# nghorbani/moshpp

Hardware: NVIDIA H100
Metric: mocap frames solved/sec (Stage-II) (higher is better)
Workload: dtype f32

## Files before the change

### moshpp_b200/csrc/mosh2_device.cuh

```cuda
#pragma once
#include <math.h>
#include <stdint.h>

#if defined(__CUDACC__) && !defined(MOSH2_EMU)
#define M2_HD __host__ __device__ __forceinline__
#define M2_D __device__ __forceinline__
#define M2_NOINLINE __device__ __noinline__
#define M2_SYNC() __syncthreads()
#define M2_WSYNC() __syncwarp()
#define M2_GPU 1
#else
#define M2_HD inline
#define M2_D inline
#define M2_NOINLINE static inline
#define M2_SYNC() ((void)0)
#define M2_WSYNC() ((void)0)
#define M2_GPU 0
#endif

#if defined(MOSH2_PROFILE) && M2_GPU
#define M2_T0() long long t_prev_ = clock64()
#define M2_TACC(slot) do { if (cta.tid == 0) { const long long t_now_ = clock64(); w.prof[(slot) + prof_base] += t_now_ - t_prev_; t_prev_ = t_now_; } } while (0)
#define M2_TRESET() do { t_prev_ = clock64(); } while (0)
#else
// ... 1450 lines not shown
                real sacc = on ? s0 + s1 : real(0);
                const real a1 = __shfl_sync(0xffffffffu, sacc, (src0 + 1) & 31), a2 = __shfl_sync(0xffffffffu, sacc, (src0 + 2) & 31);
                if (on && part == 0) out[i] = (sacc + a1) + a2;
            }
        }
        __syncthreads();
#else
        for (int i = 0; i < n; ++i) {
            real s = 0;
            for (int j = 0; j < n; ++j) s += w.A[i * d.lda + j] * v[j];
            out[i] = s;
        }
#endif
    }

    M2_D bool chol_diag(int k0, int n) {
        const int ld = d.ld;
        constexpr int NB = kCholNB;
        const int kb = (n - k0 < NB) ? n - k0 : NB;
        real *Li = w.Linv + (k0 / NB) * NB * NB;
#if M2_GPU
        {

            const int lane = cta.tid;
            real *base = w.Lm + (k0 * ld + k0);
            real Lb[NB][NB], invd[NB], x[NB];
#pragma unroll
            for (int r = 0; r < NB; ++r) {
                Vec4<real> v0, v1;
                v0.x = v0.y = v0.z = v0.w = real(0);
                v1 = v0;
                if (r < kb) {
                    v0 = ld4(base + r * ld);
                    if (r >= 4) v1 = ld4(base + r * ld + 4);
                } else {
                    if (r == 0) v0.x = real(1);
                    if (r == 1) v0.y = real(1);
                    if (r == 2) v0.z = real(1);
                    if (r == 3) v0.w = real(1);
                    if (r == 4) v1.x = real(1);
                    if (r == 5) v1.y = real(1);
                    if (r == 6) v1.z = real(1);
                    if (r == 7) v1.w = real(1);
                }
                Lb[r][0] = v0.x; Lb[r][1] = v0.y; Lb[r][2] = v0.z; Lb[r][3] = v0.w;
                Lb[r][4] = v1.x; Lb[r][5] = v1.y; Lb[r][6] = v1.z; Lb[r][7] = v1.w;
            }
            bool ok = true;
#pragma unroll
            for (int cc = 0; cc < NB; ++cc) {
                const real piv = Lb[cc][cc];
                if (!(piv > pivot_eps<real>())) ok = false;
                const real iv = r_rsqrt(piv);
                Lb[cc][cc] = piv * iv;
                invd[cc] = iv;
#pragma unroll
                for (int r = cc + 1; r < NB; ++r) Lb[r][cc] *= iv;
#pragma unroll
                for (int r = cc + 1; r < NB; ++r)
#pragma unroll
                    for (int q = cc + 1; q <= r; ++q) Lb[r][q] -= Lb[r][cc] * Lb[q][cc];
            }
            const int c = lane & (NB - 1);
#pragma unroll
            for (int r = 0; r < NB; ++r) x[r] = (r == c) ? real(1) : real(0);
#pragma unroll
            for (int pp = 0; pp < NB; ++pp) {
                x[pp] *= invd[pp];
#pragma unroll
                for (int r = pp + 1; r < NB; ++r) x[r] -= Lb[r][pp] * x[pp];
            }
            if (lane < NB) {
#pragma unroll
                for (int r = 0; r < NB; ++r) Li[r * NB + lane] = x[r];
            }
            __syncwarp();
            if (lane == 0) {
#pragma unroll
                for (int r = 0; r < NB; ++r)
                    if (r < kb) {
                        Vec4<real> v0, v1;
                        v0.x = Lb[r][0]; v0.y = r >= 1 ? Lb[r][1] : real(0); v0.z = r >= 2 ? Lb[r][2] : real(0); v0.w = r >= 3 ? Lb[r][3] : real(0);
                        *reinterpret_cast<Vec4<real> *>(base + r * ld) = v0;
                        if (r >= 4) {
                            v1.x = Lb[r][4]; v1.y = r >= 5 ? Lb[r][5] : real(0); v1.z = r >= 6 ? Lb[r][6] : real(0); v1.w = r >= 7 ? Lb[r][7] : real(0);
                            *reinterpret_cast<Vec4<real> *>(base + r * ld + 4) = v1;
                        }
                    }
            }
            return ok;
                }
#else
        {

            real Lk[NB * NB], id[NB];
            bool ok = true;
            for (int r = 0; r < kb; ++r)
                for (int cc = 0; cc <= r; ++cc) {
                    real sacc = w.Lm[(k0 + r) * ld + k0 + cc];
                    for (int p = 0; p < cc; ++p) sacc -= Lk[r * NB + p] * Lk[cc * NB + p];
                    if (cc == r) {
                        if (!(sacc > pivot_eps<real>())) { ok = false; sacc = real(1); }
                        const real sq = r_sqrt(sacc);
                        Lk[r * NB + r] = sq;
                        id[r] = real(1) / sq;
                    } else Lk[r * NB + cc] = sacc * id[cc];
                }
            for (int cc = 0; cc < kb; ++cc)
                for (int r = 0; r < kb; ++r) {
                    real v = 0;
                    if (r == cc) v = id[r];
                    else if (r > cc) {
                        real sacc = 0;
                        for (int p = cc; p < r; ++p) sacc -= Lk[r * NB + p] * Li[p * NB + cc];
                        v = sacc * id[r];
                    }
                    Li[r * NB + cc] = v;
                }
            for (int r = 0; r < kb; ++r)
                for (int cc = 0; cc <= r; ++cc) w.Lm[(k0 + r) * ld + k0 + cc] = Lk[r * NB + cc];
            for (int r = 0; r < NB; ++r)
                for (int cc = 0; cc < NB; ++cc)
                    if (r >= kb || cc >= kb) Li[r * NB + cc] = (r == cc) ? real(1) : real(0);
            if (!ok) w.isc[3] = 0;
            return ok;
                }
#endif
    }

    M2_D void chol_tile(int it, int r0, int n) {
        const int ld = d.ld;
        constexpr int NB = kCholNB;
        int ti = 0, rem = it;
        while (rem > ti) { rem -= ti + 1; ++ti; }
        const int tj = rem;
        real acc[kBS * kBS];
#pragma unroll
        for (int q = 0; q < kBS * kBS; ++q) acc[q] = 0;
#pragma unroll
        for (int cc = 0; cc < NB; ++cc) {
            const Vec4<real> av = ld4(w.Pn + cc * d.ldp + r0 + ti * kBS), bv = ld4(w.Pn + cc * d.ldp + r0 + tj * kBS);
            const real ai[4] = {av.x, av.y, av.z, av.w}, bj[4] = {bv.x, bv.y, bv.z, bv.w};
#pragma unroll
            for (int p = 0; p < kBS; ++p)
#pragma unroll
                for (int q = 0; q < kBS; ++q) acc[p * kBS + q] += ai[p] * bj[q];
        }
#pragma unroll
        for (int p = 0; p < kBS; ++p) {
            const int i = r0 + ti * kBS + p;
            if (i <= n && r0 + tj * kBS < n) {
                real *dst = w.Lm + i * ld + r0 + tj * kBS;
                Vec4<real> v = ld4(dst);
                v.x -= acc[p * kBS]; v.y -= acc[p * kBS + 1]; v.z -= acc[p * kBS + 2]; v.w -= acc[p * kBS + 3];
                *reinterpret_cast<Vec4<real> *>(dst) = v;
            }
        }
    }

    M2_D void panel_row(int i, int k0, int kb, const real *Li, int n) {
        const int ld = d.ld;
        constexpr int NB = kCholNB;
        real xr[NB];
#pragma unroll
        for (int cc = 0; cc < NB; ++cc) xr[cc] = 0;
        if (i <= n) {
            real *row = w.Lm + i * ld + k0;
            real av[NB];
            {
                const Vec4<real> a0 = ld4(row), a1 = ld4(row + 4);
                av[0] = a0.x; av[1] = a0.y; av[2] = a0.z; av[3] = a0.w; av[4] = a1.x; av[5] = a1.y; av[6] = a1.z; av[7] = a1.w;
            }
#pragma unroll
            for (int cc = 0; cc < NB; ++cc) if (cc >= kb) av[cc] = real(0);
#pragma unroll
            for (int cc = 0; cc < NB; ++cc) {
                const Vec4<real> l0 = ld4(Li + cc * NB);
                real sacc = av[0] * l0.x;
                if (cc >= 1) sacc += av[1] * l0.y;
                if (cc >= 2) sacc += av[2] * l0.z;
                if (cc >= 3) sacc += av[3] * l0.w;
                if (cc >= 4) {
                    const Vec4<real> l1 = ld4(Li + cc * NB + 4);
                    sacc += av[4] * l1.x;
                    if (cc >= 5) sacc += av[5] * l1.y;
                    if (cc >= 6) sacc += av[6] * l1.z;
                    if (cc >= 7) sacc += av[7] * l1.w;
                }
                xr[cc] = cc < kb ? sacc : real(0);
            }
            if (kb == NB) {
                Vec4<real> o0, o1;
                o0.x = xr[0]; o0.y = xr[1]; o0.z = xr[2]; o0.w = xr[3]; o1.x = xr[4]; o1.y = xr[5]; o1.z = xr[6]; o1.w = xr[7];
                *reinterpret_cast<Vec4<real> *>(row) = o0;
                *reinterpret_cast<Vec4<real> *>(row + 4) = o1;
            } else {
#pragma unroll
                for (int cc = 0; cc < NB; ++cc) if (cc < kb) row[cc] = xr[cc];
            }
        }
#pragma unroll
        for (int cc = 0; cc < NB; ++cc) w.Pn[cc * d.ldp + i] = xr[cc];
    }

    M2_D bool gauss_newton(int n) {
        const int ld = d.ld;
        constexpr int NB = kCholNB;
        M2_T0();
        CTA_FOR(i, n) {
            const real a = w.A[i * d.lda + i];
            w.ds[i] = (a > real(0)) ? real(1) / r_sqrt(a) : real(0);
        }
        M2_SYNC();
#if M2_GPU
        {
            const int lane = cta.tid & 31, warp = cta.tid >> 5, nwarp = cta.nthr >> 5;
            for (int i = warp; i < n; i += nwarp)
                for (int j = lane; j <= i; j += 32) w.Lm[i * ld + j] = w.A[i * d.lda + j] * w.ds[i] * w.ds[j];
        }
#else
        for (int i = 0; i < n; ++i)
            for (int j = 0; j <= i; ++j) w.Lm[i * ld + j] = w.A[i * d.lda + j] * w.ds[i] * w.ds[j];
#endif
        CTA_FOR(j, n) w.Lm[n * ld + j] = w.g[j] * w.ds[j];
        M2_SYNC();
        M2_TACC(11);
#if M2_GPU
        {
            const int nthr = cta.nthr;
#pragma unroll 1
            for (int k0 = -NB; k0 < n; k0 += NB) {
                bool ok = true;
                const int kb = k0 < 0 ? 0 : ((n - k0 < NB) ? n - k0 : NB);
                const int r0 = k0 < 0 ? 0 : k0 + kb;
                const real *Li = w.Linv + (k0 < 0 ? 0 : k0 / NB) * NB * NB;
                const bool trail = k0 >= 0 && r0 < n;
                if (cta.tid < 32) {
                    if (k0 >= 0) {
                        const int i = r0 + cta.tid;
                        M2_TACC(14);
                        if (cta.tid < NB && i < d.ldp) panel_row(i, k0, kb, Li, n);
                        if (trail) {
                            __threadfence_block();
                            __syncwarp();
                            asm volatile("bar.arrive 1, %0;" :: "r"(nthr) : "memory");
                            {
                                const int pr = cta.tid >> 2, q0 = (cta.tid & 3) * 2;
                                const int ii = r0 + pr, jj = r0 + q0;
                                if (ii <= n && jj < n) {
                                    real acc0 = 0, acc1 = 0;
#pragma unroll
                                    for (int cc = 0; cc < NB; ++cc) {
                                        const real pi = w.Pn[cc * d.ldp + ii];
                                        acc0 += pi * w.Pn[cc * d.ldp + jj];
                                        acc1 += pi * w.Pn[cc * d.ldp + jj + 1];
                                    }
                                    w.Lm[ii * ld + jj] -= acc0;
                                    w.Lm[ii * ld + jj + 1] -= acc1;
                                }
                            }
                            __syncwarp();
                        }
                    }
                    M2_TACC(12);
                    if (r0 < n) ok = chol_diag(r0, n);
                    M2_TACC(13);
                } else {
                    if (k0 >= 0) {
                        const int t = cta.tid - 32, nt_ = nthr - 32;
                        for (int i = r0 + NB + t; i < d.ldp; i += nt_) panel_row(i, k0, kb, Li, n);
                        if (trail) {
                            asm volatile("bar.sync 1, %0;" :: "r"(nthr) : "memory");
                            const int R = n + 1 - r0, ntl = (R + kBS - 1) / kBS, ntri = ntl * (ntl + 1) / 2;
                            for (int it = 3 + t; it < ntri; it += nt_) chol_tile(it, r0, n);
                        }
                    }
                }
                if (__syncthreads_or(!ok)) return false;
            }
            M2_TACC(14);
        }
#else
        w.isc[3] = 1;
        chol_diag(0, n);
        if (w.isc[3] == 0) return false;
        for (int k0 = 0; k0 < n; k0 += NB) {
            const int kb = (n - k0 < NB) ? n - k0 : NB;
            const real *Li = w.Linv + (k0 / NB) * NB * NB;
            for (int i = k0 + kb; i < d.ldp; ++i) panel_row(i, k0, kb, Li, n);
            const int r0 = k0 + kb, R = r0 < n ? n + 1 - r0 : 0;
            if (R > 0) {
                const int nt = (R + kBS - 1) / kBS, ntri = nt * (nt + 1) / 2;
                for (int it = 0; it < ntri; ++it) chol_tile(it, r0, n);
                chol_diag(r0, n);
                if (w.isc[3] == 0) return false;
            }
        }
#endif
#if M2_GPU
        if (cta.tid < 128) {
            const int tid = cta.tid;
            for (int i = tid; i < n; i += 128) w.tmp[i] = w.Lm[n * ld + i];
            asm volatile("bar.sync 2, 128;" ::: "memory");
#pragma unroll 1
            for (int k0 = ((n - 1) / NB) * NB; k0 >= 0; k0 -= NB) {
                const int kb = (n - k0 < NB) ? n - k0 : NB;
                const real *Li = w.Linv + (k0 / NB) * NB * NB;
                real zv[NB], y[NB], Lr[NB][NB];
                {
                    const Vec4<real> z0 = ld4(w.tmp + k0), z1 = ld4(w.tmp + k0 + 4);
                    zv[0] = z0.x; zv[1] = z0.y; zv[2] = z0.z; zv[3] = z0.w; zv[4] = z1.x; zv[5] = z1.y; zv[6] = z1.z; zv[7] = z1.w;
                }
#pragma unroll
                for (int cc = 1; cc < NB; ++cc) if (cc >= kb) zv[cc] = real(0);
#pragma unroll
                for (int pp = 0; pp < NB; ++pp) {
                    const Vec4<real> l0 = ld4(Li + pp * NB);
                    Lr[pp][0] = l0.x; Lr[pp][1] = l0.y; Lr[pp][2] = l0.z; Lr[pp][3] = l0.w;
                    if (pp >= 4) {
                        const Vec4<real> l1 = ld4(Li + pp * NB + 4);
                        Lr[pp][4] = l1.x; Lr[pp][5] = l1.y; Lr[pp][6] = l1.z; Lr[pp][7] = l1.w;
                    }
                }
#pragma unroll
                for (int cc = 0; cc < NB; ++cc) {
                    real sacc = 0;
#pragma unroll
                    for (int pp = cc; pp < NB; ++pp) sacc += Lr[pp][cc] * zv[pp];
                    y[cc] = sacc;
                }
                for (int i = tid; i < k0; i += 128) {
                    real zi = w.tmp[i];
#pragma unroll
                    for (int cc = 0; cc < NB; ++cc) if (cc < kb) zi -= w.Lm[(k0 + cc) * ld + i] * y[cc];
                    w.tmp[i] = zi;
                }
                asm volatile("bar.sync 2, 128;" ::: "memory");
                if (tid == 0) {
                    if (kb == NB) {
                        Vec4<real> o0, o1;
                        o0.x = y[0]; o0.y = y[1]; o0.z = y[2]; o0.w = y[3]; o1.x = y[4]; o1.y = y[5]; o1.z = y[6]; o1.w = y[7];
                        *reinterpret_cast<Vec4<real> *>(w.tmp + k0) = o0;
                        *reinterpret_cast<Vec4<real> *>(w.tmp + k0 + 4) = o1;
                    } else {
#pragma unroll
                        for (int cc = 0; cc < NB; ++cc) if (cc < kb) w.tmp[k0 + cc] = y[cc];
                    }
                }
            }
            asm volatile("bar.sync 2, 128;" ::: "memory");
            for (int i = tid; i < n; i += 128) w.dgn[i] = w.tmp[i] * w.ds[i];
        }
#else
        const int wl = cta.nthr < 32 ? cta.nthr : 32;
        if (cta.tid < wl) {
            const int lane = cta.tid;
            for (int i = lane; i < n; i += wl) w.tmp[i] = w.Lm[n * ld + i];
            M2_WSYNC();
            for (int k0 = ((n - 1) / NB) * NB; k0 >= 0; k0 -= NB) {
                const int kb = (n - k0 < NB) ? n - k0 : NB;
                const real *Li = w.Linv + (k0 / NB) * NB * NB;
                real zv[NB], y[NB];
#pragma unroll
                for (int cc = 0; cc < NB; ++cc) zv[cc] = cc < kb ? w.tmp[k0 + cc] : real(0);
#pragma unroll
                for (int cc = 0; cc < NB; ++cc) {
                    real sacc = 0;
#pragma unroll
                    for (int pp = cc; pp < NB; ++pp) sacc += Li[pp * NB + cc] * zv[pp];
                    y[cc] = sacc;
                }
                for (int i = lane; i < k0; i += wl) {
                    real zi = w.tmp[i];
#pragma unroll
                    for (int cc = 0; cc < NB; ++cc) if (cc < kb) zi -= w.Lm[(k0 + cc) * ld + i] * y[cc];
                    w.tmp[i] = zi;
                }
                M2_WSYNC();
                if (lane == 0) {
#pragma unroll
                    for (int cc = 0; cc < NB; ++cc) if (cc < kb) w.tmp[k0 + cc] = y[cc];
                }
                M2_WSYNC();
            }
            for (int i = lane; i < n; i += wl) w.dgn[i] = w.tmp[i] * w.ds[i];
        }
#endif
        M2_SYNC();
        M2_TACC(15);
        return true;
    }

    M2_D void stage_tables(int which) {
        const int *free = which ? static_cast<const int *>(w.c_free2) : static_cast<const int *>(w.c_free1);
        const int n = which ? m.n2 : m.n1;
        CTA_FOR(i, d.NX) w.colmap[i] = -1;
        CTA_FOR(i, d.nJ) w.jlist[i] = 0;
        M2_SYNC();
        CTA_FOR(i, n) {
            const int fv = free[i];
            w.colmap[fv] = i;
            int src;
            if (fv < 3) src = -1 - fv;
            else if (fv < 3 + m.body_dof) { src = fv - 3; w.jlist[(fv - 3) / 3] = 1; }
            else if (fv < 3 + d.PR) src = -4;
            else src = d.PF + (fv - 3 - d.PR);
            w.colsrc[i] = src;
        }
        M2_SYNC();
        if (cta.tid == 0) {
            int hf = 0;
            for (int b = 0; b < m.hb_n; ++b) {
                bool any = false;
                for (int r = m.hb[b].r0; r < m.hb[b].r1; ++r) any = any || w.colmap[3 + m.body_dof + r] >= 0;
                if (any) {
                    hf = 1;
                    for (int q = m.hb[b].q0; q < m.hb[b].q1; ++q) w.jlist[(m.body_dof + q) / 3] = 1;
                }
            }
            int cnt = 0;
            for (int j = 0; j < d.nJ; ++j) if (w.jlist[j]) w.jlist[cnt++] = j;
            w.st_meta[2 * which] = cnt;
            w.st_meta[2 * which + 1] = hf;
        }
        M2_SYNC();
        CTA_FOR(i, d.NX) w.st_colmap[which * d.NX + i] = w.colmap[i];
        CTA_FOR(i, n) w.st_colsrc[which * d.n2 + i] = w.colsrc[i];
        CTA_FOR(i, d.nJ) w.st_jlist[which * d.nJ + i] = w.jlist[i];
        M2_SYNC();
    }

    M2_D void stage_setup(const StepCfg<real> &c) {
        ++n_min;
        const int which = c.free == static_cast<const int *>(w.c_free2) ? 1 : 0;
        CTA_FOR(i, d.NX) w.colmap[i] = w.st_colmap[which * d.NX + i];
        CTA_FOR(i, c.n) w.colsrc[i] = w.st_colsrc[which * d.n2 + i];
        CTA_FOR(i, d.nJ) w.jlist[i] = w.st_jlist[which * d.nJ + i];
        njl = w.st_meta[2 * which];
        hand_free = w.st_meta[2 * which + 1] != 0;
        M2_SYNC();
    }

    M2_D void solve_frame(int f, bool emit, bool first, bool fingers, bool dyn, bool face, bool light) {
        const Options &o = job.opt;
        const real e1 = real(1e-15), e2 = real(1e-15);
        enum { OP_PROCRUSTES, OP_BEGIN, OP_TRIAL, OP_OUTPUT };
        int op = first ? OP_PROCRUSTES : OP_BEGIN;
        int stage = first ? 0 : (light ? 4 : 3);
        if (lin_f >= 0) stage = job.lin_step == 2 ? 4 : 3;
        const int maxit = light ? 1 : o.maxiter;
        StepCfg<real> c;
        c.free = w.c_free1; c.n = m.n1; c.velo = has_velo; c.poseH = false; c.dm_terms = false; c.extrap = false; c.face = false;
        c.wp = 0; c.e3 = real(o.e3_first);
        bool need_setup = !first;
        real sse0 = 0, delta = 0, alpha = 0, nsd = 0, ngn2 = 0, gn_sd = 0, nstep = 0, npn = 0, gd = 0, dAd = 0;
        bool done = false, in_iter = false, have_gn = false, gn_ok = true;
        int iter = 0;
        M2_T0();
        while (true) {
            if (need_setup) {
                M2_TACC(25);
                c.free = w.c_free1; c.n = m.n1; c.poseH = false; c.dm_terms = false; c.extrap = false; c.face = false;
                if (stage < 3) {
                    c.wp = wp_frame * (stage == 0 ? real(10) : (stage == 1 ? real(5) : real(1)));
                    c.e3 = real(o.e3_first);
                } else {
                    c.wp = wp_frame;
                    c.e3 = real(o.e3);
                    if (stage == 4) { c.free = w.c_free2; c.n = m.n2; c.poseH = fingers; c.dm_terms = dyn; c.extrap = has_extrap; c.face = face; }
                }
                stage_setup(c);
                need_setup = false;
                M2_TACC(20);
            }
            const int n = c.n;
            {
                const bool reuse = op != OP_TRIAL && fwd_at_x && (fwd_has_prior || !(c.wp > real(0)));
                M2_TACC(25);
                eval(op == OP_TRIAL ? w.xt : w.x, c, reuse);
                M2_TRESET();
                if (!reuse) fwd_has_prior = c.wp > real(0);
                fwd_at_x = op != OP_TRIAL;
            }
            if (lin_f >= 0) {
                CTA_FOR(i, 3 * d.M) { job.markers_sim[size_t(f) * 3 * d.M + i] = w.mk[i]; if (job.lin_r) job.lin_r[size_t(f) * 3 * d.M + i] = w.rm[i]; }
                CTA_FOR(i, N_ERR) job.errs[size_t(f) * N_ERR + i] = w.sc[1 + i];
                if (job.lin_vp) CTA_FOR(i, 3 * d.S) job.lin_vp[size_t(f) * 3 * d.S + i] = w.vp[i];
                if (job.lin_mode < 2) break;
            }
            if (op == OP_PROCRUSTES) {
                procrustes();
                fwd_at_x = false;
                op = OP_BEGIN;
                need_setup = true;
                continue;
            }
            if (op == OP_OUTPUT) break;
            bool do_build = false, improved = false;
            if (op == OP_BEGIN) {
                sse0 = w.sc[0];
                delta = real(o.delta_0);
                done = false; in_iter = false; iter = 0;
                do_build = true;
            } else {
                const real sse1 = w.sc[0];
                real rho = sse0 - sse1;
                improved = rho > real(0) || rho >= -accept_slack<real>() * sse0;
                if (rho > real(0)) rho = rho / (real(2) * gd - dAd);
                if (improved) {
                    CTA_FOR(i, d.NX) w.x[i] = w.xt[i];
                    fwd_at_x = true;
                    M2_SYNC();
                    if (c.e3 > real(0) && (sse0 - sse1) / sse0 < c.e3) done = true;
                    else { do_build = true; sse0 = sse1; }
                }
                if (rho > real(0.9)) { const real cand = real(2.5) * nstep; if (cand > delta) delta = cand; }
                else if (rho < real(0.05)) delta *= real(0.25);
                if (delta <= e2 * npn) done = true;
                if (done || improved) {
                    in_iter = false;
                    if (!done && iter >= maxit) { done = true; if (!light) frame_flags |= ST_MAXITER; }
                }
            }
            M2_TACC(21);
            if (do_build && !done) build(w.x, c);
            M2_TRESET();
            if (lin_f >= 0) {
                CTA_FOR(idx, n * n) { const int i = idx / n, j = idx - i * n; job.lin_A[size_t(f) * n * n + idx] = w.A[i * d.lda + j]; }
                CTA_FOR(i, n) job.lin_g[size_t(f) * n + i] = w.g[i];
                break;
            }
            if (op == OP_BEGIN) {
                real sq[1] = {0};
                CTA_FOR(i, n) sq[0] += w.g[i] * w.g[i];
                cta_reduce<real, 1>(cta, sq, w.red);
                if (r_sqrt(sq[0]) < e1) done = true;
            }
            if (!done) {
                if (!in_iter) {
                    ++iter;
                    ++n_iter;
                    symv(w.g, w.Ag, n);
                    real r2[2] = {0, 0};
                    CTA_FOR(i, n) { r2[0] += w.g[i] * w.g[i]; r2[1] += w.g[i] * w.Ag[i]; }
                    cta_reduce<real, 2>(cta, r2, w.red);
                    alpha = r2[0] / r2[1];
                    nsd = alpha * r_sqrt(r2[0]);
                    have_gn = false; gn_ok = true;
                    in_iter = true;
                }
                int kind;
                real beta = 0, scale_sd = 0;
                if (nsd >= delta) { kind = 0; scale_sd = delta / nsd * alpha; }
                else {
                    if (!have_gn) {
                        M2_TACC(22);
                        gn_ok = gauss_newton(n);
                        M2_TRESET();
                        have_gn = true;
                        if (gn_ok) {
                            real q[2] = {0, 0};
                            CTA_FOR(i, n) { q[0] += w.dgn[i] * w.dgn[i]; q[1] += w.dgn[i] * w.g[i]; }
                            cta_reduce<real, 2>(cta, q, w.red);
                            ngn2 = q[0];
                            gn_sd = alpha * q[1];
                        } else frame_flags |= ST_GN_FALLBACK;
                    }
                    if (!gn_ok) { kind = 0; scale_sd = alpha; }
                    else if (r_sqrt(ngn2) <= delta) kind = 1;
                    else {
                        kind = 2;
                        const real dsq = delta * delta, sd2 = nsd * nsd;
                        const real diff2 = ngn2 - real(2) * gn_sd + sd2;
                        const real pnow = diff2 * dsq + gn_sd * gn_sd - ngn2 * sd2;
                        beta = (dsq - sd2) / ((gn_sd - sd2) + r_sqrt(pnow));
                    }
                }
                CTA_FOR(i, n) {
                    real v;
                    if (kind == 0) v = scale_sd * w.g[i];
                    else if (kind == 1) v = w.dgn[i];
                    else v = alpha * w.g[i] + beta * (w.dgn[i] - alpha * w.g[i]);
                    w.d[i] = v;
                }
                M2_SYNC();
                symv(w.d, w.tmp, n);
                real q[4] = {0, 0, 0, 0};
                CTA_FOR(i, n) {
                    q[0] += w.d[i] * w.d[i];
                    q[1] += w.g[i] * w.d[i];
                    q[2] += w.d[i] * w.tmp[i];
                    const real pv = w.x[c.free[i]];
                    q[3] += pv * pv;
                }
                cta_reduce<real, 4>(cta, q, w.red);
                nstep = r_sqrt(q[0]); gd = q[1]; dAd = q[2]; npn = r_sqrt(q[3]);
                if (nstep <= e2 * npn) done = true;
                else {
                    CTA_FOR(i, d.NX) w.xt[i] = w.x[i];
                    M2_SYNC();
                    CTA_FOR(i, n) w.xt[c.free[i]] += w.d[i];
                    M2_SYNC();
                    op = OP_TRIAL;
                    M2_TACC(23);
                    continue;
                }
            }
            if (stage < 4) { ++stage; op = OP_BEGIN; need_setup = true; continue; }
            if (!emit) break;
            op = OP_OUTPUT;
        }
        if (cta.tid == 0 && job.totals) {
#if M2_GPU
            atomicAdd(job.totals + 0, n_iter); atomicAdd(job.totals + 1, n_eval);
            atomicAdd(job.totals + 2, n_build); atomicAdd(job.totals + 3, n_min);
            if (emit) {
                atomicAdd(job.totals + 4, n_iter); atomicAdd(job.totals + 5, n_eval);
                atomicAdd(job.totals + 6, n_build); atomicAdd(job.totals + 7, n_min);
            }
#else
            job.totals[0] += n_iter; job.totals[1] += n_eval; job.totals[2] += n_build; job.totals[3] += n_min;
            if (emit) { job.totals[4] += n_iter; job.totals[5] += n_eval; job.totals[6] += n_build; job.totals[7] += n_min; }
#endif
        }
        if (emit && resuming) {
            real dm[1] = {0};
            if (job.status[f] & ST_SOLVED) {
                const int nbody = m.body_dof < 66 ? m.body_dof : 66;
                CTA_FOR(i, d.PR) {
                    real e = r_abs(w.x[3 + i] - job.pose[size_t(f) * d.PR + i]);
                    if (i >= nbody) e *= real(0.1);
                    if (e > dm[0]) dm[0] = e;
                }
                CTA_FOR(i, 3) { const real e = real(10) * r_abs(w.x[i] - job.trans[size_t(f) * 3 + i]); if (e > dm[0]) dm[0] = e; }
            } else dm[0] = real(1);
            cta_max(dm);
            resume_diff = dm[0];
        }
        if (emit) {
            CTA_FOR(i, d.PF) job.fullpose[size_t(f) * d.PF + i] = w.fullpose[i];
            CTA_FOR(i, d.PR) job.pose[size_t(f) * d.PR + i] = w.x[3 + i];
            CTA_FOR(i, 3) job.trans[size_t(f) * 3 + i] = w.x[i];
            if (job.dmpls) CTA_FOR(i, d.nd) job.dmpls[size_t(f) * d.nd + i] = w.x[3 + d.PR + i];
            CTA_FOR(i, 3 * d.M) job.markers_sim[size_t(f) * 3 * d.M + i] = w.mk[i];
            CTA_FOR(i, N_ERR) job.errs[size_t(f) * N_ERR + i] = w.sc[1 + i];
            if (cta.tid == 0) {
                job.status[f] = ST_SOLVED | frame_flags | (has_velo ? ST_HAS_VELO : 0) | (has_extrap ? ST_HAS_EXTRAP : 0);
                job.counters[4 * f + 0] = n_iter;
                job.counters[4 * f + 1] = n_eval;
                job.counters[4 * f + 2] = n_build;
// ... 288 lines not shown
```

Measured before the change: 131,100.

## Process two blocks per iteration in backward triangular solve to halve barriers

The blocked backward substitution now handles two NB-blocks per loop iteration. Every thread redundantly computes the second block's partial update and y values, then applies both blocks' updates to the remaining rows in a single pass. This halves the number of 128-thread named barriers and the passes over w.tmp. In exchange each thread does extra redundant work (NB*NB loads from Lm per pair), and Linv entries are now read straight from memory rather than through preloaded vector registers.

```diff
diff --git a/moshpp_b200/csrc/mosh2_device.cuh b/moshpp_b200/csrc/mosh2_device.cuh
--- a/moshpp_b200/csrc/mosh2_device.cuh
+++ b/moshpp_b200/csrc/mosh2_device.cuh
@@ -1776,50 +1776,65 @@
             const int tid = cta.tid;
             for (int i = tid; i < n; i += 128) w.tmp[i] = w.Lm[n * ld + i];
             asm volatile("bar.sync 2, 128;" ::: "memory");
-#pragma unroll 1
-            for (int k0 = ((n - 1) / NB) * NB; k0 >= 0; k0 -= NB) {
-                const int kb = (n - k0 < NB) ? n - k0 : NB;
-                const real *Li = w.Linv + (k0 / NB) * NB * NB;
-                real zv[NB], y[NB], Lr[NB][NB];
-                {
-                    const Vec4<real> z0 = ld4(w.tmp + k0), z1 = ld4(w.tmp + k0 + 4);
-                    zv[0] = z0.x; zv[1] = z0.y; zv[2] = z0.z; zv[3] = z0.w; zv[4] = z1.x; zv[5] = z1.y; zv[6] = z1.z; zv[7] = z1.w;
-                }
-#pragma unroll
-                for (int cc = 1; cc < NB; ++cc) if (cc >= kb) zv[cc] = real(0);
-#pragma unroll
-                for (int pp = 0; pp < NB; ++pp) {
-                    const Vec4<real> l0 = ld4(Li + pp * NB);
-                    Lr[pp][0] = l0.x; Lr[pp][1] = l0.y; Lr[pp][2] = l0.z; Lr[pp][3] = l0.w;
-                    if (pp >= 4) {
-                        const Vec4<real> l1 = ld4(Li + pp * NB + 4);
-                        Lr[pp][4] = l1.x; Lr[pp][5] = l1.y; Lr[pp][6] = l1.z; Lr[pp][7] = l1.w;
-                    }
-                }
+            auto block_y = [&](int k, const real (&zv)[NB], real (&y)[NB]) {
+                const real *Li = w.Linv + (k / NB) * NB * NB;
 #pragma unroll
                 for (int cc = 0; cc < NB; ++cc) {
                     real sacc = 0;
 #pragma unroll
-                    for (int pp = cc; pp < NB; ++pp) sacc += Lr[pp][cc] * zv[pp];
+                    for (int pp = cc; pp < NB; ++pp) sacc += Li[pp * NB + cc] * zv[pp];
                     y[cc] = sacc;
                 }
-                for (int i = tid; i < k0; i += 128) {
-                    real zi = w.tmp[i];
-#pragma unroll
-                    for (int cc = 0; cc < NB; ++cc) if (cc < kb) zi -= w.Lm[(k0 + cc) * ld + i] * y[cc];
-                    w.tmp[i] = zi;
+            };
+            auto store_y = [&](int k, int kb, const real (&y)[NB]) {
+                if (kb == NB) {
+                    Vec4<real> o0, o1;
+                    o0.x = y[0]; o0.y = y[1]; o0.z = y[2]; o0.w = y[3]; o1.x = y[4]; o1.y = y[5]; o1.z = y[6]; o1.w = y[7];
+                    *reinterpret_cast<Vec4<real> *>(w.tmp + k) = o0;
+                    *reinterpret_cast<Vec4<real> *>(w.tmp + k + 4) = o1;
+                } else {
+#pragma unroll
+                    for (int cc = 0; cc < NB; ++cc) if (cc < kb) w.tmp[k + cc] = y[cc];
+                }
+            };
+#pragma unroll 1
+            for (int k1 = ((n - 1) / NB) * NB; k1 >= 0; k1 -= 2 * NB) {
+                const int kb = (n - k1 < NB) ? n - k1 : NB;
+                const int k0 = k1 - NB;
+                real zv[NB], y1[NB], y0[NB];
+                {
+                    const Vec4<real> z0 = ld4(w.tmp + k1), z1 = ld4(w.tmp + k1 + 4);
+                    zv[0] = z0.x; zv[1] = z0.y; zv[2] = z0.z; zv[3] = z0.w; zv[4] = z1.x; zv[5] = z1.y; zv[6] = z1.z; zv[7] = z1.w;
+                }
+#pragma unroll
+                for (int cc = 1; cc < NB; ++cc) if (cc >= kb) zv[cc] = real(0);
+                block_y(k1, zv, y1);
+                if (k0 >= 0) {
+                    {
+                        const Vec4<real> z0 = ld4(w.tmp + k0), z1 = ld4(w.tmp + k0 + 4);
+                        zv[0] = z0.x; zv[1] = z0.y; zv[2] = z0.z; zv[3] = z0.w; zv[4] = z1.x; zv[5] = z1.y; zv[6] = z1.z; zv[7] = z1.w;
+                    }
+#pragma unroll
+                    for (int r = 0; r < NB; ++r) {
+                        real zi = zv[r];
+#pragma unroll
+                        for (int cc = 0; cc < NB; ++cc) if (cc < kb) zi -= w.Lm[(k1 + cc) * ld + k0 + r] * y1[cc];
+                        zv[r] = zi;
+                    }
+                    block_y(k0, zv, y0);
+                    for (int i = tid; i < k0; i += 128) {
+                        real zi = w.tmp[i];
+#pragma unroll
+                        for (int cc = 0; cc < NB; ++cc) if (cc < kb) zi -= w.Lm[(k1 + cc) * ld + i] * y1[cc];
+#pragma unroll
+                        for (int cc = 0; cc < NB; ++cc) zi -= w.Lm[(k0 + cc) * ld + i] * y0[cc];
+                        w.tmp[i] = zi;
+                    }
                 }
                 asm volatile("bar.sync 2, 128;" ::: "memory");
                 if (tid == 0) {
-                    if (kb == NB) {
-                        Vec4<real> o0, o1;
-                        o0.x = y[0]; o0.y = y[1]; o0.z = y[2]; o0.w = y[3]; o1.x = y[4]; o1.y = y[5]; o1.z = y[6]; o1.w = y[7];
-                        *reinterpret_cast<Vec4<real> *>(w.tmp + k0) = o0;
-                        *reinterpret_cast<Vec4<real> *>(w.tmp + k0 + 4) = o1;
-                    } else {
-#pragma unroll
-                        for (int cc = 0; cc < NB; ++cc) if (cc < kb) w.tmp[k0 + cc] = y[cc];
-                    }
+                    store_y(k1, kb, y1);
+                    if (k0 >= 0) store_y(k0, NB, y0);
                 }
             }
             asm volatile("bar.sync 2, 128;" ::: "memory");
```

Result: faster. 135,200 (median of 6 runs) (+3.1%).
